# LuckyLYM/Zebra

Measured on AMD Instinct MI355X. Metric: temporal edges/sec embedded (k=20, 2-layer), higher is better.
Workload: dtype f64+f32

## Files before the change

include/zebra_amd.h:

```cpp
#ifndef ZEBRA_AMD_H
#define ZEBRA_AMD_H

#include <stdint.h>

#ifdef __cplusplus
extern "C" {
#endif

#define ZT_OK 0
#define ZT_ERR_ARG (-1)
#define ZT_ERR_RANGE (-2)
#define ZT_ERR_HIP (-3)
#define ZT_ERR_UNSUPPORTED (-4)
#define ZT_ERR_TIMEOUT (-5)

#define ZT_MAX_K 63
#define ZT_MAX_K_WIDE 255

const char *zt_last_error(void);
const char *zt_version(void);

int zt_stream_create_masked(void **stream_out, int32_t cu_lo, int32_t cu_hi);
int zt_stream_destroy(void *stream);

#define ZT_CHOICE_AGGREGATE 0
#define ZT_CHOICE_EMBED_OUT 1
#define ZT_CHOICE_GRU 2
#define ZT_CHOICE_MESSAGES 3
#define ZT_CHOICE_TPPR_CHAIN 4
#define ZT_CHOICE_TPPR_PREPASS 5
#define ZT_CHOICE_GROUP_RELEASE 6
#define ZT_CHOICE_COUNT 7
#define ZT_AGG_GENERIC 1
#define ZT_OUT_TILED 1
#define ZT_OUT_LATENCY 2
#define ZT_OUT_PERSIST 3
#define ZT_GRU_TILE 1
#define ZT_GRU_SPLIT 2
#define ZT_CHAIN_SINGLE 1
#define ZT_CHAIN_PAIRED 2
#define ZT_CHAIN_SPINE 3
#define ZT_CHAIN_DUO 4
#define ZT_PREPASS_LAUNCHES 1
#define ZT_PREPASS_COOP 2
#define ZT_RELEASE_MEMBER 1
#define ZT_RELEASE_LAUNCH 2
#define ZT_RELEASE_LAUNCH_FULL 3
#define ZT_MSG_ONE 1
#define ZT_MSG_TWO 2
int zt_set_kernel_choice(int32_t which, int32_t value);

int zt_profile_enable(int on);
int zt_profile_reset(void);
int zt_profile_read(const char *name, int64_t *count, double *total_ms);


typedef struct zt_tppr zt_tppr;

int zt_tppr_create(zt_tppr **out, int64_t num_nodes, int32_t k, int32_t n_tppr,
                   const double *alpha_host, const double *beta_host);
int zt_tppr_destroy(zt_tppr *h);
int zt_tppr_set_device_share(zt_tppr *h, int32_t n_processes);
int zt_tppr_chain_stats(zt_tppr *h, int64_t *out5, void *stream);

int zt_tppr_reset(zt_tppr *h, void *stream);

int zt_tppr_copy(zt_tppr *dst, const zt_tppr *src, void *stream);

int zt_tppr_stream(zt_tppr *h, const int32_t *nodes_dev, const double *ts_dev,
                   const int64_t *eidx_dev, int64_t B, int32_t n_roles,
                   int32_t emit, int32_t model, int32_t *out_nodes_dev,
                   int32_t *out_eidx_dev, float *out_dt_dev, float *out_w_dev,
                   uint64_t plan_token, void *stream);

int zt_tppr_plan(zt_tppr *h, const int32_t *nodes_dev, const int64_t *eidx_dev,
                 int64_t B, int32_t n_roles, int32_t model, uint64_t *token_out,
                 void *stream);

int zt_tppr_status(zt_tppr *h, void *stream);

int zt_tppr_export(zt_tppr *h, int32_t m, int32_t *len_host, double *norm_host,
                   int64_t *eidx_host, int64_t *node_host, double *ts_host,
                   double *w_host);
int zt_tppr_export_rows(zt_tppr *h, int32_t m, const int64_t *ids_host, int64_t n,
                        int32_t *len_host, double *norm_host, int64_t *eidx_host,
                        int64_t *node_host, double *ts_host, double *w_host);
// ... 266 lines not shown
```

zebra_amd/_capi.py:

```python
import ctypes as C
import os

import torch

_HERE = os.path.dirname(os.path.abspath(__file__))
LIB_PATH = os.path.join(_HERE, "lib", "libzebra_amd.so")

ZT_OK = 0
ZT_ERR_ARG, ZT_ERR_RANGE, ZT_ERR_HIP, ZT_ERR_UNSUPPORTED, ZT_ERR_TIMEOUT = -1, -2, -3, -4, -5

SYMBOLS = [
    "zt_last_error", "zt_version", "zt_set_kernel_choice", "zt_profile_enable", "zt_profile_reset", "zt_profile_read", "zt_stream_create_masked", "zt_stream_destroy",
    "zt_tppr_create", "zt_tppr_destroy", "zt_tppr_set_device_share", "zt_tppr_chain_stats", "zt_tppr_reset", "zt_tppr_copy", "zt_tppr_stream", "zt_tppr_plan", "zt_tppr_status",
    "zt_tppr_export", "zt_tppr_export_rows", "zt_tppr_import", "zt_tppr_import_rows",
    "zt_csr_build", "zt_csr_from_sorted", "zt_csr_size", "zt_csr_export", "zt_csr_destroy", "zt_csr_find_before", "zt_pruned_topk", "zt_pruned_topk_multi",
    "zt_embed_workspace_bytes", "zt_embed", "zt_project_table_bytes", "zt_project_memory", "zt_agg_train_forward", "zt_agg_backward_workspace_bytes", "zt_agg_train_backward", "zt_agg_train_supported", "zt_pipeline_create", "zt_pipeline_destroy", "zt_pipeline_main_stream", "zt_pipeline_update", "zt_pipeline_step", "zt_pipeline_step_ahead", "zt_pipeline_set_group",
    "zt_store_messages", "zt_store_messages_range", "zt_gru_workspace_bytes", "zt_gru_rows_offset", "zt_gru_update", "zt_gemm_f32", "zt_colsum_f32", "zt_overlay_rows", "zt_overlay_rows_backward", "zt_gru_train_workspace_bytes", "zt_gru_train_forward", "zt_gru_train_backward", "zt_pipeline_set_stats", "zt_pipeline_outstanding", "zt_pack_rows", "zt_scatter_rows", "zt_attention_workspace_bytes", "zt_temporal_attention",
    "zt_affinity_workspace_bytes", "zt_affinity", "zt_link_metrics", "zt_pipeline_set_scoring", "zt_pipeline_last_scores", "zt_pipeline_run",
    "zt_exchange_unique_id", "zt_exchange_create", "zt_exchange_set_tables", "zt_exchange_destroy", "zt_pipeline_set_exchange",
    "zt_rnn_update", "zt_rnn_train_forward", "zt_rnn_train_backward", "zt_pipeline_set_cell",
]


CHOICE_AGGREGATE, CHOICE_EMBED_OUT, CHOICE_GRU, CHOICE_MESSAGES, CHOICE_TPPR_CHAIN, CHOICE_TPPR_PREPASS = 0, 1, 2, 3, 4, 5
CHOICE_GROUP_RELEASE = 6
RELEASE_MEMBER, RELEASE_LAUNCH, RELEASE_LAUNCH_FULL = 1, 2, 3
PREPASS_LAUNCHES, PREPASS_COOP = 1, 2
CHAIN_SINGLE, CHAIN_PAIRED, CHAIN_SPINE, CHAIN_DUO = 1, 2, 3, 4
AGG_GENERIC = 1
OUT_TILED, OUT_LATENCY, OUT_PERSIST = 1, 2, 3
GRU_TILE, GRU_SPLIT = 1, 2
CELL_GRU, CELL_RNN = 0, 1
MSG_ONE, MSG_TWO = 1, 2


def set_kernel_choice(which, value):
    check(lib().zt_set_kernel_choice(C.c_int32(which), C.c_int32(value)), "zt_set_kernel_choice")
    _choices[which] = value


_choices = {}


def kernel_choice(which):
    return _choices.get(which, 0)


class RowTables(C.Structure):
    _fields_ = [("ptr", C.c_void_p * 8), ("width", C.c_int32 * 8), ("n", C.c_int32)]


class EmbedWeights(C.Structure):
    _fields_ = [(n, C.c_void_p) for n in ("fc1_w", "fc1_b", "fc2_w", "fc2_b", "fc1s_w", "fc1s_b", "fc2s_w",
                                          "fc2s_b", "time_w")]


class AttnWeights(C.Structure):
    _fields_ = [(n, C.c_void_p) for n in ("q_w", "k_w", "v_w", "in_b", "out_w", "out_b", "m1_w", "m1_b", "m2_w", "m2_b")]


class AffinityWeights(C.Structure):
    _fields_ = [(n, C.c_void_p) for n in ("fc1_w", "fc1_b", "fc2_w", "fc2_b")]


class GruWeights(C.Structure):
    _fields_ = [(n, C.c_void_p) for n in ("w_ih", "w_hh", "b_ih", "b_hh")]


class PipelineDesc(C.Structure):
    _fields_ = [("tppr", C.c_void_p), ("csr", C.c_void_p), ("width", C.c_int32), ("depth", C.c_int32),
                ("alpha", C.c_double * 16), ("beta", C.c_double * 16),
                ("memory", C.c_void_p), ("last_update", C.c_void_p), ("messages", C.c_void_p), ("msg_ts", C.c_void_p),
                ("flags", C.c_void_p), ("scratch", C.c_void_p), ("efeat", C.c_void_p),
                ("num_nodes", C.c_int64), ("num_edges", C.c_int64),
                ("D", C.c_int32), ("F", C.c_int32), ("T", C.c_int32), ("M", C.c_int32), ("k", C.c_int32),
                ("ew", EmbedWeights), ("gw", GruWeights),
                ("embed_ws", C.c_void_p), ("gru_ws", C.c_void_p), ("proj_table", C.c_void_p), ("status", C.c_void_p),
                ("max_B", C.c_int64)]


XCHG_RCCL, XCHG_SHM = 1, 2

# ... 96 lines not shown
```

zebra_amd/csrc/aggregate.hip:

```cpp
#include "common.hpp"
#include "embed_out_body.hpp"

using namespace zt;

namespace {

constexpr int MAX_MT = 5;
constexpr int MAX_MT_BIG = 16;
constexpr int MAX_MT_BIG_WIDE = 8;
constexpr int LDS_BUDGET = 150 * 1024;

__host__ __device__ inline int round_up(int x, int m) { return (x + m - 1) / m * m; }

#ifdef ZT_AGG_STAMP
__device__ unsigned long long g_agg[8];
#define AGG_STAMP(i) do { if (threadIdx.x == 0) { const long long t__ = clock64(); atomicAdd(&g_agg[i], (unsigned long long)(t__ - t_prev__)); t_prev__ = t__; } } while (0)
#else
#define AGG_STAMP(i) do { } while (0)
#endif

__global__ void k_pad_matrix(const float *__restrict__ W, int ld, int c0, int rows, int cols, float *__restrict__ Wp,
                             int rows_p, int cols_p)
{
    const int i = blockIdx.x * blockDim.x + threadIdx.x;
// ... 766 lines not shown
                            acc[b] = __builtin_amdgcn_mfma_f32_16x16x4f32(A_cur[u], Breg[b][st0 + u], acc[b], 0, 0, 0);
                }
#pragma unroll
                for (int u = 0; u < 2; ++u) {
                    const int st = st0 + u;
                    if (!(a > 0 && st < REG_NB)) continue;
                    const int b = st;
                    float part = 0.f;
#pragma unroll
                    for (int j = 0; j < 4; ++j) {
                        float v = accv[b][j] + ((DBG & 2) ? 0.f : Pv[ap & 1][b][j]);
                        v = v > 0.f ? v : 0.f;
                        part += (DBG & 2) ? v : v * wn_prv[j];
                    }
                    if (DBG & 2) {
                        Hloc[q_lo][b] += part;
                    } else {
                        const int pi = __float_as_int(part);
                        const auto h = __builtin_amdgcn_permlane32_swap(pi, pi, false, false);
                        const auto lo = __builtin_amdgcn_permlane16_swap(h[0], h[0], false, false);
                        const auto hi = __builtin_amdgcn_permlane16_swap(h[1], h[1], false, false);
                        const float pg[4] = {__int_as_float(lo[0]), __int_as_float(lo[1]), __int_as_float(hi[0]), __int_as_float(hi[1])};
#pragma unroll
                        for (int g = 0; g < 4; ++g) {
                            const int q = (16 * ap + 4 * g) / KK;
                            if (q < RQ) Hloc[q][b] += pg[g];
                        }
                    }
                    asm volatile("" : "+v"(Hloc[q_lo][b]));
                    if (q_hi != q_lo && q_hi < RQ) asm volatile("" : "+v"(Hloc[q_hi][b]));
                }
                if (a >= 1 && a <= 3 && st0 == REG_NB + 1 && !(DBG & 4)) load_P(a + 1);
                __builtin_amdgcn_sched_barrier(0);
            }
        }
#pragma unroll
        for (int q = 0; q < RQ; ++q) {
            if (g4 == (q & 3) && q < nq) {
                float *hrow = H + ((size_t)m * N + q0 + q) * D;
#pragma unroll
                for (int b = 0; b < REG_NB; ++b)
                    if (16 * b + r16 < D) hrow[16 * b + r16] = Hloc[q][b];
            }
        }
        wave_sync();
    }
#ifdef ZT_DIAG
    if (DBG && lane == 0 && blockIdx.x * AGG_WAVES + wave < 1024) {
        unsigned long long *o = g_regclk + 4 * (blockIdx.x * AGG_WAVES + wave);
        o[0] = __builtin_amdgcn_s_memtime() - clk0; o[1] = wall0; o[2] = __builtin_amdgcn_s_memrealtime();
        o[3] = wall_in;
    }
#endif
}


constexpr int EO3_NT = 7, EO3_KC = 7, EO3_DP = 112, EO3_LDY = 116;
constexpr int EO3_FRAG = EO3_NT * EO3_KC * 256;

__device__ __forceinline__ void eo3_fill(float *Wl, const float *__restrict__ Wp, int tid)
{
    constexpr int PER = (EO3_NT * EO3_KC * 64 + 255) / 256;
    f32x4 v[PER];
#pragma unroll
    for (int q = 0; q < PER; ++q) {
        const int idx = tid + q * 256, frag = idx >> 6, ln = idx & 63;
        const int b = frag / EO3_KC, c = frag - b * EO3_KC;
        v[q] = idx < EO3_NT * EO3_KC * 64
                   ? *reinterpret_cast<const f32x4 *>(Wp + (size_t)(16 * b + (ln & 15)) * EO3_DP + 16 * c + 4 * (ln >> 4))
                   : f32x4{0.f, 0.f, 0.f, 0.f};
    }
#pragma unroll
    for (int q = 0; q < PER; ++q) {
        const int idx = tid + q * 256;
        if (idx < EO3_NT * EO3_KC * 64) reinterpret_cast<f32x4 *>(Wl)[idx] = v[q];
    }
}

template <int HG>
__global__ __launch_bounds__(AGG_THREADS, 1) void k_embed_out3(
    const float *__restrict__ memory, long long num_nodes, const int *__restrict__ nodes, long long N, int D, int M,
    const float *__restrict__ H, const float *__restrict__ S, const float *__restrict__ fc2_p,
    const float *__restrict__ fc2_b, const float *__restrict__ fc1s_p, const float *__restrict__ fc1s_b,
    const float *__restrict__ fc2s_p, const float *__restrict__ fc2s_b, float *__restrict__ out, int *status, int n_src)
{
    extern __shared__ __attribute__((aligned(16))) char smem[];
    float *W0 = reinterpret_cast<float *>(smem);
    const int tid = threadIdx.x, lane = tid & 63, wave = tid >> 6, r16 = lane & 15, g4 = lane >> 4;
    const int OW = D * (M + 1);
    const long long tiles = (N + 15) / 16;
    const f32x4 zero4 = {0.f, 0.f, 0.f, 0.f};
    bool cin[EO3_KC];
#pragma unroll
    for (int c = 0; c < EO3_KC; ++c) cin[c] = 16 * c + 4 * g4 < D;
    const f32x4 *Wf0 = reinterpret_cast<const f32x4 *>(W0) + lane;

    if ((int)blockIdx.x < n_src) {
        float *W1 = W0 + EO3_FRAG;
        float *Y = W1 + EO3_FRAG + wave * 16 * EO3_LDY;
        eo3_fill(W0, fc1s_p, tid);
        eo3_fill(W1, fc2s_p, tid);
        float b1v[EO3_NT], b2v[EO3_NT];
#pragma unroll
        for (int b = 0; b < EO3_NT; ++b) {
            b1v[b] = 16 * b + r16 < D ? fc1s_b[16 * b + r16] : 0.f;
            b2v[b] = 16 * b + r16 < D ? fc2s_b[16 * b + r16] : 0.f;
// ... 192 lines not shown
{
    const int lda = Kp + 4;
    int mt = max_mt;
    while (mt > 1 && ((size_t)mt * 16 * lda * 4 + (size_t)mt * 16 * 16) > (size_t)LDS_BUDGET) --mt;
    int rq = (mt * 16) / k;
    if (rq < 1) {
        mt = (k + 15) / 16;
        rq = 1;
        if (mt > max_mt || ((size_t)mt * 16 * lda * 4 + (size_t)mt * 16 * 16) > (size_t)LDS_BUDGET) return false;
    }
    mt = (rq * k + 15) / 16;
    if ((size_t)mt * 16 * (Dp + 1) * 4 > (size_t)mt * 16 * lda * 4) return false;
    *lda_out = lda; *mt_out = mt; *rq_out = rq;
    *lds_out = (size_t)mt * 16 * lda * 4 + (size_t)mt * 16 * 16 + (size_t)T * 4;
    return true;
}

bool split_fits(int D, int F, int T, int k) { return k <= ZT_MAX_K_WIDE && fc1_agg_split_rows(D, F, T) > 0; }

bool make_plan(int64_t N, int D, int F, int T, int M, int k, EmbedPlan &p)
{
    if (!width_supported(D)) return false;
    const int K1 = D + F + T;
    p.Dp = round_up(D, 16);
    p.K1p = round_up(K1, 16);
    const bool big = k > MAX_MT * 16;
    const int max_mt = big ? (p.Dp > 16 * NTW * AGG_WAVES ? MAX_MT_BIG_WIDE : MAX_MT_BIG) : MAX_MT;
    const bool full_ok = tile_shape(p.K1p, p.Dp, k, T, &p.lda, &p.mt, &p.rq, &p.lds, max_mt);
    if (!full_ok) { p.mt = 0; p.rq = 1; p.lda = p.K1p + 4; p.lds = 0; }
    p.K2p = round_up(F + T, 16);
    p.mt2 = 0;
    if (!(full_ok || big) || !tile_shape(p.K2p, p.Dp, k, T, &p.lda2, &p.mt2, &p.rq2, &p.lds2, max_mt)) p.mt2 = 0;
    if (p.mt == 0 && p.mt2 == 0 && !split_fits(D, F, T, k)) return false;
    size_t o = 0;
    auto take = [&](size_t bytes) { size_t r = o; o += (bytes + 255) & ~(size_t)255; return r; };
    p.off_w1p = take((size_t)p.Dp * p.K1p * 4);
    p.off_fc2t = take((size_t)p.Dp * p.Dp * 4);
    p.off_fc1st = take((size_t)p.Dp * p.Dp * 4);
    p.off_fc2st = take((size_t)p.Dp * p.Dp * 4);
    p.off_w1t = take((size_t)p.Dp * p.K2p * 4);
    p.off_wm = take((size_t)p.Dp * p.Dp * 4);
    p.hg = fc1_agg_wide_supported(D, F, T, k) ? k / 4 : 1;
    p.off_wl = take(p.hg > 1 ? fc1_agg_wide_weight_bytes() : 0);
    p.off_wfrag = take((size_t)REG_FRAG_GROUPS * 64 * 4 * 4);
    p.off_H = take((size_t)M * N * D * 4 * p.hg);
    p.off_S = take((size_t)M * N * 4);
    p.total = o;
    return true;
}

KernelPlan plan_kernels(int64_t N, int D, int F, int T, int M, int k, bool have_table, bool training, int agg_choice,
                        int out_choice, EmbedPlan &p)
{
    KernelPlan kp{AggKernel::unsupported, OutForm::tiled, Refusal::shape, 0, 0, 0, 0, 1};
    static_assert(16 * NTW * AGG_WAVES == 128 && 16 * NTW_WIDE * AGG_WAVES == MAX_D, "the N-tiles cover D <= 128 / D <= 256");
    if (!make_plan(N, D, F, T, M, k, p)) return kp;
    const bool big = k > MAX_MT * 16;
    const bool tab = have_table && !training && p.mt2 > 0;
    const bool special = tab && agg_choice != ZT_AGG_GENERIC;
    if (training ? (big || p.mt == 0) : (!tab && p.mt == 0)) {
        if (!split_fits(D, F, T, k)) { kp.refusal = Refusal::no_split; return kp; }
        kp.agg = AggKernel::split;
    } else if (special && p.hg > 1) {
        kp.agg = AggKernel::wide;
    } else if (special && D == 100 && T == 100 && F <= 4 && (k == 20 || k == 40) && p.K2p == 112) {
        kp.agg = AggKernel::reg;
    } else if (special && D == 100 && T == 100 && p.mt2 == 5 && (k == 10 || k == 20 || k == 40)) {
        kp.agg = AggKernel::d100;
    } else if (tab) {
        kp.agg = big ? AggKernel::tiled_table_big : AggKernel::tiled_table;
    } else {
        kp.agg = big ? AggKernel::tiled_full_big : AggKernel::tiled_full;
    }
    if (kp.agg == AggKernel::d100 || kp.agg == AggKernel::tiled_table || kp.agg == AggKernel::tiled_table_big) {
        kp.lds = p.lds2; kp.rq = p.rq2; kp.mt = p.mt2; kp.lda = p.lda2;
    } else if (kp.agg == AggKernel::tiled_full || kp.agg == AggKernel::tiled_full_big) {
        kp.lds = p.lds; kp.rq = p.rq; kp.mt = p.mt; kp.lda = p.lda;
    }
    kp.hg = kp.agg == AggKernel::wide ? p.hg : 1;
    if (kp.hg != 1 && kp.hg != 5 && kp.hg != 10) { kp.agg = AggKernel::unsupported; kp.refusal = Refusal::groups; return kp; }
    kp.refusal = Refusal::none;
    if (D % 4 == 0 && (p.Dp == 112 || p.Dp == 128) && (out_choice == ZT_OUT_LATENCY || (out_choice == 0 && N <= 1024)))
        kp.out = OutForm::latency;
    else if (D % 4 == 0 && p.Dp == EO3_DP && (out_choice == ZT_OUT_PERSIST || (out_choice == 0 && N >= 8192)))
        kp.out = OutForm::persist;
    return kp;
}

}

KernelPlan zt::embed_kernel_plan(int64_t N, int D, int F, int T, int M, int k, bool have_table, bool training, int agg_choice,
                                 int out_choice)
{
    EmbedPlan p;
    return plan_kernels(N, D, F, T, M, k, have_table, training, agg_choice, out_choice, p);
}

#ifdef ZT_AGG_STAMP
extern "C" int zt_debug_agg(unsigned long long *host, int reset)
{
    ZT_HIP(hipDeviceSynchronize());
    ZT_HIP(hipMemcpyFromSymbol(host, HIP_SYMBOL(g_agg), sizeof(unsigned long long) * 8));
    if (reset) { unsigned long long z[8] = {0}; ZT_HIP(hipMemcpyToSymbol(HIP_SYMBOL(g_agg), z, sizeof(z))); }
    return ZT_OK;
}
#endif

#ifdef ZT_DIAG
extern "C" int zt_debug_regclk(unsigned long long *host)
{
    ZT_HIP(hipDeviceSynchronize());
    ZT_HIP(hipMemcpyFromSymbol(host, HIP_SYMBOL(g_regclk), sizeof(unsigned long long) * 4 * 1024));
    return ZT_OK;
}
#endif

extern "C" int64_t zt_embed_workspace_bytes(int64_t N, int32_t D, int32_t F, int32_t T, int32_t M, int32_t k)
{
    EmbedPlan p;
// ... 83 lines not shown
    if (N == 0) return ZT_OK;
    if (!nodes_dev || !nbr_dev || !eix_dev || !dt_dev || !w_dev || !out_dev || !workspace_dev) {
        set_error("zt_embed: NULL buffer");
        return ZT_ERR_ARG;
    }
    EmbedPlan p;
    const KernelPlan kp = plan_kernels(N, D, F, T, M, k, proj_table_dev != nullptr, false, kernel_choice(ZT_CHOICE_AGGREGATE),
                                       kernel_choice(ZT_CHOICE_EMBED_OUT), p);
    if (kp.refusal == Refusal::shape) {
        set_error("zt_embed: D=%d F=%d T=%d k=%d outside the supported shapes (D <= 128, or a multiple of 4 up to %d; one query "
                  "row of k neighbours must fit the %d KB LDS tile)", D, F, T, k, MAX_D, LDS_BUDGET / 1024);
        return ZT_ERR_UNSUPPORTED;
    }
    hipStream_t s = (hipStream_t)stream;
    char *ws = reinterpret_cast<char *>(workspace_dev);
    float *H = reinterpret_cast<float *>(ws + p.off_H);
    float *S = reinterpret_cast<float *>(ws + p.off_S);
    if (!weights_ready) {
        ZT_PROF_BEGIN(s, P_EMBED_PREP);
        embed_prepare(wt, D, F, T, p, ws, s);
        ZT_PROF_END(s, P_EMBED_PREP);
    }
    if (kp.refusal == Refusal::no_split) {
        set_error("zt_embed: k=%d needs the projected table (a query row's [memory | ef | time] tile does not fit %d KB of LDS, "
                  "nor does a chunk of it)", k, LDS_BUDGET / 1024);
        return ZT_ERR_UNSUPPORTED;
    }
    if (kp.refusal == Refusal::groups) { set_error("zt_embed: %d partial-sum groups per row", kp.hg); return ZT_ERR_UNSUPPORTED; }
    const bool waits_inside = kp.agg == AggKernel::wide || kp.agg == AggKernel::reg;
    if (gate != nullptr && gate->word != nullptr && !waits_inside) {
        const int rc = zt::member_gate_launch(*gate, status_dev, s);
        if (rc != ZT_OK) return rc;
    }
    const dim3 tile_grid((unsigned)(kp.rq > 0 ? (N + kp.rq - 1) / kp.rq : 0), (unsigned)M);
    const bool wide = p.Dp > 16 * NTW * AGG_WAVES;
    auto tiled = [&](decltype(&k_fc1_agg<false>) fn, const float *rows, int ld, size_t w_off, int Kp) {
        ZT_HIP(set_dynamic_lds(reinterpret_cast<const void *>(fn), kp.lds));
        fn<<<tile_grid, AGG_THREADS, kp.lds, s>>>(rows, efeat_dev, wt->time_w, num_nodes, num_edges, ld, F, T, N, k, kp.rq, kp.mt,
                                                  kp.lda, nbr_dev, eix_dev, dt_dev, w_dev, reinterpret_cast<const float *>(ws + w_off),
                                                  Kp, wt->fc1_b, H, S, status_dev, D, nullptr, nullptr, 0u, 0u, 0u, 1.f);
        return ZT_OK;
    };
    auto reg = [&](decltype(&k_fc1_agg_reg<20>) fn) {
        const long long rq = 80 / k, tiles = ((N + rq - 1) / rq) * M;
        long long wgs = (tiles + AGG_WAVES - 1) / AGG_WAVES;
        const int cus = stream_cu_count(s);
        if (wgs > cus) wgs = cus;
        fn<<<(unsigned)wgs, AGG_THREADS, 0, s>>>(proj_table_dev, efeat_dev, wt->time_w, num_nodes, num_edges, F, N, M, nbr_dev, eix_dev,
                                                 dt_dev, w_dev, reinterpret_cast<const float *>(ws + p.off_wfrag), wt->fc1_b, H, S,
                                                 status_dev, gate ? gate->word : nullptr, gate ? gate->target : 0,
                                                 gate ? gate->latch : nullptr);
        return ZT_OK;
    };
    ZT_PROF_BEGIN(s, P_FC1_AGG);
    int rc = ZT_OK;
    switch (kp.agg) {
    case AggKernel::wide:
        rc = fc1_agg_wide_launch(proj_table_dev, efeat_dev, wt->time_w, num_nodes, num_edges, N, M, k, nbr_dev, eix_dev, dt_dev,
                                 w_dev, reinterpret_cast<const float *>(ws + p.off_wl), wt->fc1_b, H, S, status_dev,
                                 stream_cu_count(s), s, gate);
        break;
    case AggKernel::reg:
#ifdef ZT_DIAG
        {
            static const int dbg = getenv("ZT_AGG_DBG") ? atoi(getenv("ZT_AGG_DBG")) : 0;
            if (k == 20 && dispatch<1, 2, 6, 7, 8>(dbg, [&](auto DB) { return reg(k_fc1_agg_reg<20, DB>); }) == ZT_OK) break;
        }
#endif
        rc = dispatch<20, 40>(k, [&](auto KK) { return reg(k_fc1_agg_reg<KK>); });
        break;
    case AggKernel::d100:
        rc = dispatch<10, 20, 40>(k, [&](auto KK) {
            ZT_HIP(set_dynamic_lds(reinterpret_cast<const void *>(k_fc1_agg_d100<KK>), kp.lds));
            k_fc1_agg_d100<KK><<<tile_grid, AGG_THREADS, kp.lds, s>>>(proj_table_dev, efeat_dev, wt->time_w, num_nodes, num_edges, F, N,
                                                                     kp.lda, nbr_dev, eix_dev, dt_dev, w_dev,
                                                                     reinterpret_cast<const float *>(ws + p.off_w1t), p.K2p, wt->fc1_b,
                                                                     H, S, status_dev);
            return ZT_OK;
        });
        break;
    case AggKernel::tiled_table:
        rc = tiled(wide ? k_fc1_agg<true, MAX_MT, NTW_WIDE> : k_fc1_agg<true>, proj_table_dev, p.Dp, p.off_w1t, p.K2p);
        break;
    case AggKernel::tiled_table_big:
        rc = tiled(wide ? k_fc1_agg<true, MAX_MT_BIG_WIDE, NTW_WIDE> : k_fc1_agg<true, MAX_MT_BIG>, proj_table_dev, p.Dp, p.off_w1t,
                   p.K2p);
        break;
    case AggKernel::tiled_full: rc = tiled(wide ? k_fc1_agg<false, MAX_MT, NTW_WIDE> : k_fc1_agg<false>, memory_dev, D, p.off_w1p, p.K1p); break;
    case AggKernel::tiled_full_big:
        rc = tiled(wide ? k_fc1_agg<false, MAX_MT_BIG_WIDE, NTW_WIDE> : k_fc1_agg<false, MAX_MT_BIG>, memory_dev, D, p.off_w1p, p.K1p);
        break;
    case AggKernel::split:
        rc = fc1_agg_split_launch(memory_dev, nullptr, nullptr, efeat_dev, wt->time_w, num_nodes, num_edges, D, F, T, N, M, k,
                                  nbr_dev, eix_dev, dt_dev, w_dev, reinterpret_cast<const float *>(ws + p.off_w1p), p.K1p,
                                  wt->fc1_b, H, S, status_dev, 0.f, 0ull, s);
        break;
    case AggKernel::unsupported: break;
    }
    if (rc != ZT_OK) return rc;
    ZT_PROF_END(s, P_FC1_AGG);
    if (mid_wait != nullptr) ZT_HIP(hipStreamWaitEvent(s, mid_wait, 0));
    const EmbedOutArgs E{memory_dev, num_nodes, nodes_dev, N, D, M, H, S,
                         reinterpret_cast<const float *>(ws + p.off_fc2t), wt->fc2_b,
                         reinterpret_cast<const float *>(ws + p.off_fc1st), wt->fc1s_b,
                         reinterpret_cast<const float *>(ws + p.off_fc2st), wt->fc2s_b, out_dev, status_dev};
    const long long tiles = (N + 15) / 16;
    const zt::embed_out_deferred od{true, E, kp.hg, kp.out, kp.out == OutForm::latency ? (int)(tiles < 256 ? tiles : 256) : 0, nullptr};
    if (defer != nullptr && kp.out != OutForm::persist) {
        int *latch = defer->latch;
        *defer = od;
        defer->latch = latch;
        ZT_LAUNCH_CHECK();
        return ZT_OK;
    }
    ZT_PROF_BEGIN(s, P_EMBED_OUT);
    rc = zt::embed_out_launch(od, s);
    if (rc != ZT_OK) return rc;
    ZT_PROF_END(s, P_EMBED_OUT);
    ZT_LAUNCH_CHECK();
    return ZT_OK;
}

// ... 125 lines not shown
```

zebra_amd/csrc/common.hpp:

```cpp
#pragma once

#include <hip/hip_runtime.h>

#include <cstdint>
#include <cstdio>
#include <cstdlib>
#include <type_traits>

#include "../../include/zebra_amd.h"

namespace zt {

void set_error(const char *fmt, ...);

enum ProfId { P_PREPASS = 0, P_STREAM, P_CLEANUP, P_PRUNE, P_EMBED_PREP, P_FC1_AGG, P_EMBED_OUT, P_STORE_MSG, P_GRU,
              P_SCORE, P_EXCHANGE, P_COUNT };
extern bool g_prof_on;
void prof_begin(hipStream_t s, int id);
void prof_end(hipStream_t s, int id);
int tppr_stream_ex(zt_tppr *h, const int32_t *nodes_dev, const double *ts_dev, const int64_t *eidx_dev, int64_t B,
                   int32_t n_roles, int32_t emit, int32_t model, int32_t *out_nodes_dev, int32_t *out_eidx_dev,
                   float *out_dt_dev, float *out_w_dev, uint64_t plan_token, void *stream, bool plan_ordered,
                   hipEvent_t *done_out, int32_t sub_B, int32_t *member_done_dev = nullptr);
constexpr int TPPR_MAX_MEMBERS = 8;
constexpr int TPPR_MEMBER_WORDS = TPPR_MAX_MEMBERS + 1;
struct EmbedOutArgs {
    const float *memory;
    long long num_nodes;
    const int *nodes;
    long long N;
    int D, M;
    const float *H, *S, *fc2_p, *fc2_b, *fc1s_p, *fc1s_b, *fc2s_p, *fc2s_b;
    float *out;
    int *status;
};
enum class AggKernel { unsupported, reg, wide, d100, tiled_table, tiled_full, tiled_table_big, tiled_full_big, split };
enum class OutForm { tiled, latency, persist };
enum class Refusal { none, shape, no_split, groups };
struct KernelPlan {
    AggKernel agg;
    OutForm out;
    Refusal refusal;
    size_t lds;
    int rq, mt, lda;
    int hg;
};
KernelPlan embed_kernel_plan(int64_t N, int D, int F, int T, int M, int k, bool have_table, bool training, int agg_choice,
                             int out_choice);
enum class MsgKernel { one, two };
enum class GruForm { none, tile, split };
enum class OutLaunch { none, front, fused_tile, fused_split };
enum class MemRefusal { none, arg, d_large, msg_wide };
struct HeldOut {
    bool present;
    OutForm form;
    int hg, D, M, gx;
    long long N;
    bool same_memory;
};
struct MemoryPlan {
    MsgKernel msg;
    GruForm gru;
    OutLaunch out;
    MemRefusal refusal;
    size_t lds, lds2, lds_f;
    int gru_tiles, NTg;
    int n_src_wgs, n_nb_wgs, out_tiles;
    unsigned grid;
    unsigned target, participants;
};
MemoryPlan memory_kernel_plan(int64_t max_rows, int D, int msg_dim, int F, int T, int gru_choice, int msg_choice,
                              const HeldOut &held);
struct embed_out_deferred {
    bool valid;
    EmbedOutArgs args;
    int hg;
    OutForm form;
    int gx;
    int *latch;
};
int embed_out_launch(const embed_out_deferred &d, void *stream);
int gru_update_ex(float *memory_dev, float *last_update_dev, const float *messages_dev, const float *msg_ts_dev,
                  uint8_t *flags_dev, int64_t num_nodes, int32_t D, int32_t msg_dim, const int32_t *ids_dev, int64_t n_ids,
                  const int32_t *n_ids_dev, const zt_gru_weights *wt, void *workspace_dev, int32_t weights_ready,
                  const float *wm_p, float *proj_table, void *stream, bool counter_zeroed = false, bool select_done = false,
                  embed_out_deferred *fuse = nullptr, int cell = ZT_CELL_GRU);
int store_messages_ex(const float *memory_dev, const float *last_update_dev, const float *efeat_dev, const float *time_w_dev,
                      int64_t num_nodes, int64_t num_edges, int32_t D, int32_t F, int32_t T, const int32_t *src_dev,
                      const int32_t *dst_dev, const double *ts_dev, const int64_t *eidx_dev, int64_t B, int64_t pos_lo,
                      int64_t pos_hi, float *messages_dev, float *msg_ts_dev, uint8_t *flags_dev, int32_t *scratch_dev,
                      int32_t *uniq_ids_dev, int32_t *n_uniq_dev, int32_t *status_dev, int32_t *zero_word_dev, void *stream,
                      bool *zeroed_out = nullptr, bool set_flags = true);
struct member_gate {
    const int32_t *word;
    int32_t target;
    int *latch;
};
int member_gate_launch(const member_gate &g, int32_t *status_dev, void *stream);
// ... 256 lines not shown
```

Before: 13.39 million.

## Add shared-entry register aggregation kernel that dedups repeated neighbor slots across roles

Adds a new fc1 aggregate kernel for D=100, T=100, k=20/40 that groups two query roles per wave-unit, detects neighbor slots in the second role identical to live slots in the first, and computes the fc1 MFMA only for unique live entries, compacted via ballot. Results are staged in LDS and reused in the weighted sum, with prefetching of the next unit's indices and edge features overlapping compute. It becomes the default when M<=2, with a new choice value to fall back to the plain register kernel. The added LDS staging, ballot compaction and a persistent grid capped at the CU count add overhead that pays off only when many entries are zero-weight or duplicated.

```diff
diff --git a/include/zebra_amd.h b/include/zebra_amd.h
--- a/include/zebra_amd.h
+++ b/include/zebra_amd.h
@@ -32,6 +32,7 @@
 #define ZT_CHOICE_GROUP_RELEASE 6
 #define ZT_CHOICE_COUNT 7
 #define ZT_AGG_GENERIC 1
+#define ZT_AGG_REG_PLAIN 2
 #define ZT_OUT_TILED 1
 #define ZT_OUT_LATENCY 2
 #define ZT_OUT_PERSIST 3
diff --git a/zebra_amd/_capi.py b/zebra_amd/_capi.py
--- a/zebra_amd/_capi.py
+++ b/zebra_amd/_capi.py
@@ -28,6 +28,7 @@
 PREPASS_LAUNCHES, PREPASS_COOP = 1, 2
 CHAIN_SINGLE, CHAIN_PAIRED, CHAIN_SPINE, CHAIN_DUO = 1, 2, 3, 4
 AGG_GENERIC = 1
+AGG_REG_PLAIN = 2
 OUT_TILED, OUT_LATENCY, OUT_PERSIST = 1, 2, 3
 GRU_TILE, GRU_SPLIT = 1, 2
 CELL_GRU, CELL_RNN = 0, 1
diff --git a/zebra_amd/csrc/aggregate.hip b/zebra_amd/csrc/aggregate.hip
--- a/zebra_amd/csrc/aggregate.hip
+++ b/zebra_amd/csrc/aggregate.hip
@@ -842,6 +842,305 @@
         o[3] = wall_in;
     }
 #endif
+}
+
+constexpr int REGS_PITCH = 100;
+constexpr int REGS_MAX_M = 2;
+struct __attribute__((aligned(16))) RegsLds {
+    int nb[80], ei[80];
+    float dt[80], w[80], ef[80 * 4];
+    int e_nb[80];
+    float e_dt[80], e_ef[80 * 4];
+    int ent[80];
+    float sum[4];
+    float stage[80 * REGS_PITCH];
+};
+static_assert(sizeof(RegsLds) % 16 == 0 && AGG_WAVES * sizeof(RegsLds) <= 160 * 1024, "four waves' buffers in one CU's LDS");
+
+template <int KK>
+__global__ __launch_bounds__(AGG_THREADS, 1) void k_fc1_agg_regs(
+    const float *__restrict__ P, const float *__restrict__ efeat, const float *__restrict__ time_w, long long num_nodes,
+    long long num_edges, int F, long long N, int M, const int *__restrict__ nbr, const int *__restrict__ eix,
+    const float *__restrict__ dt, const float *__restrict__ w, const float *__restrict__ Wfrag,
+    const float *__restrict__ b1, float *__restrict__ H, float *__restrict__ S, int *status,
+    const int *gate_word, int gate_target, int *gate_latch)
+{
+    constexpr int D = 100, T = 100, DP = 112, ROWS = 80, RQ = ROWS / KK, PITCH = REGS_PITCH;
+    static_assert(KK % 4 == 0 && ROWS % KK == 0 && RQ % REGS_MAX_M == 0, "groups of 4 slots must not straddle query rows");
+    extern __shared__ __attribute__((aligned(16))) char smem[];
+    const int lane = threadIdx.x & 63, wave = threadIdx.x >> 6;
+    const int r16 = lane & 15, g4 = lane >> 4;
+    RegsLds &L = reinterpret_cast<RegsLds *>(smem)[wave];
+
+    float Breg[REG_NB][REG_NS];
+    {
+        const f32x4 *Wf = reinterpret_cast<const f32x4 *>(Wfrag) + lane;
+        constexpr int HB = REG_FRAG_GROUPS / 2;
+#pragma unroll
+        for (int half = 0; half < 2; ++half) {
+            f32x4 v[HB];
+#pragma unroll
+            for (int i = 0; i < HB; ++i) v[i] = Wf[(half * HB + i) * 64];
+            __builtin_amdgcn_sched_barrier(0);
+#pragma unroll
+            for (int i = 0; i < HB; ++i)
+#pragma unroll
+                for (int e = 0; e < 4; ++e) {
+                    const int q = 4 * (half * HB + i) + e;
+                    if (q < REG_NB * REG_NS) asm volatile("v_accvgpr_write_b32 %0, %1" : "=a"(Breg[q / REG_NS][q % REG_NS]) : "v"(v[i][e]));
+                }
+            __builtin_amdgcn_sched_barrier(0);
+        }
+    }
+    float freq[REG_NS];
+#pragma unroll
+    for (int st = 0; st < REG_NS; ++st) {
+        const int kc = 4 * st + g4 - F;
+        freq[st] = (kc >= 0 && kc < T) ? time_w[kc] : 0.f;
+    }
+    float bias[REG_NB];
+#pragma unroll
+    for (int b = 0; b < REG_NB; ++b) bias[b] = (16 * b + r16) < D ? b1[16 * b + r16] : 0.f;
+
+    const bool two = M == 2;
+    const int UQ = two ? RQ / 2 : RQ;
+    const long long n_units = (N + UQ - 1) / UQ;
+    const long long stride = (long long)gridDim.x * AGG_WAVES;
+    long long unit = (long long)blockIdx.x * AGG_WAVES + wave;
+
+    int pf_nb[2] = {0, 0}, pf_ei[2] = {0, 0};
+    float pf_dt[2] = {0.f, 0.f}, pf_w[2] = {0.f, 0.f};
+    auto fetch = [&](long long u) {
+        const long long q0 = u * UQ;
+        int ln = lane;
+        asm volatile("" : "+v"(ln));
+#pragma unroll
+        for (int h = 0; h < 2; ++h) {
+            const int row = h * 64 + ln;
+            const int r = row / KK, j = row - r * KK;
+            const int m = (two && r >= RQ / 2) ? 1 : 0, q = r - m * UQ;
+            const bool in = (h == 0 || lane < ROWS - 64) && q0 + q < N;
+            const size_t ix = in ? (((size_t)m * N + q0 + q) * KK + j) : 0;
+            pf_nb[h] = in ? nbr[ix] : 0;
+            pf_ei[h] = in ? eix[ix] : 0;
+            pf_dt[h] = in ? dt[ix] : 0.f;
+            pf_w[h] = in ? w[ix] : 0.f;
+        }
+    };
+    float pf_ef[2][4] = {{0.f, 0.f, 0.f, 0.f}, {0.f, 0.f, 0.f, 0.f}};
+    auto fetch_ef = [&]() {
+#pragma unroll
+        for (int h = 0; h < 2; ++h) {
+            const int ei = pf_ei[h];
+            const bool ok = ei >= 0 && ei < num_edges && (h == 0 || lane < ROWS - 64);
+#pragma unroll
+            for (int c = 0; c < 4; ++c) pf_ef[h][c] = (ok && c < F) ? efeat[(size_t)ei * F + c] : 0.f;
+        }
+    };
+    member_gate_enter(gate_word, gate_target, status, gate_latch);
+    if (unit < n_units) { fetch(unit); fetch_ef(); }
+
+#pragma nounroll
+    for (; unit < n_units; unit += stride) {
+        const long long q0 = unit * UQ;
+        int nbv[2], eiv[2];
+#pragma unroll
+        for (int h = 0; h < 2; ++h) {
+            const int row = h * 64 + lane;
+            nbv[h] = pf_nb[h]; eiv[h] = pf_ei[h];
+            if (h == 0 || lane < ROWS - 64) {
+                if (nbv[h] < 0 || nbv[h] >= num_nodes || eiv[h] < 0 || eiv[h] >= num_edges) { atomicExch(status, ZT_ERR_RANGE); nbv[h] = 0; eiv[h] = 0; }
+                L.nb[row] = nbv[h]; L.ei[row] = eiv[h]; L.dt[row] = pf_dt[h]; L.w[row] = pf_w[h];
+                *reinterpret_cast<f32x4 *>(L.ef + 4 * row) = f32x4{pf_ef[h][0], pf_ef[h][1], pf_ef[h][2], pf_ef[h][3]};
+            }
+        }
+        wave_sync();
+        if (lane < RQ) {
+            f32x4 wv[KK / 4];
+#pragma unroll
+            for (int j = 0; j < KK / 4; ++j) wv[j] = *reinterpret_cast<const f32x4 *>(L.w + lane * KK + 4 * j);
+            float sm = 0.f;
+#pragma unroll
+            for (int j = 0; j < KK; ++j) sm += wv[j / 4][j % 4];
+            L.sum[lane] = sm;
+            const int m = (two && lane >= RQ / 2) ? 1 : 0, q = lane - m * UQ;
+            if (q0 + q < N) S[(size_t)m * N + q0 + q] = (sm == 0.f) ? 0.f : 1.f;
+        }
+        wave_sync();
+        float wn[2] = {0.f, 0.f};
+#pragma unroll
+        for (int h = 0; h < 2; ++h) {
+            const int row = h * 64 + lane;
+            if (h == 0 || lane < ROWS - 64) {
+                const float qs = L.sum[row / KK];
+                wn[h] = (qs == 0.f) ? 0.f : pf_w[h] / qs;
+                L.w[row] = wn[h];
+            }
+        }
+        wave_sync();
+        if (two && lane < ROWS / 2) {
+            const int slot = ROWS / 2 + lane, base = (lane / KK) * KK;
+            const int mn = L.nb[slot], me = L.ei[slot], md = __float_as_int(L.dt[slot]);
+            int mt = -1;
+#pragma unroll
+            for (int jj = KK / 4 - 1; jj >= 0; --jj) {
+                const int4 n4 = *reinterpret_cast<const int4 *>(L.nb + base + 4 * jj);
+                const int4 e4 = *reinterpret_cast<const int4 *>(L.ei + base + 4 * jj);
+                const int4 d4 = *reinterpret_cast<const int4 *>(L.dt + base + 4 * jj);
+                const f32x4 w4 = *reinterpret_cast<const f32x4 *>(L.w + base + 4 * jj);
+                if (n4.w == mn && e4.w == me && d4.w == md && w4[3] != 0.f) mt = base + 4 * jj + 3;
+                if (n4.z == mn && e4.z == me && d4.z == md && w4[2] != 0.f) mt = base + 4 * jj + 2;
+                if (n4.y == mn && e4.y == me && d4.y == md && w4[1] != 0.f) mt = base + 4 * jj + 1;
+                if (n4.x == mn && e4.x == me && d4.x == md && w4[0] != 0.f) mt = base + 4 * jj;
+            }
+            L.ent[slot] = mt;
+        }
+        wave_sync();
+        bool live[2], isE[2];
+        int match[2], ent[2];
+#pragma unroll
+        for (int h = 0; h < 2; ++h) {
+            const int slot = h * 64 + lane;
+            const bool valid = h == 0 || lane < ROWS - 64;
+            live[h] = valid && wn[h] != 0.f;
+            match[h] = (two && valid && slot >= ROWS / 2 && live[h]) ? L.ent[slot] : -1;
+            isE[h] = live[h] && match[h] < 0;
+        }
+        const unsigned long long mask0 = __ballot(isE[0]), mask1 = __ballot(isE[1]);
+        const int n0 = __popcll(mask0), n_ent = n0 + __popcll(mask1);
+        const int n_mt = n_ent > 16 ? (n_ent + 15) >> 4 : 1;
+        ent[0] = (int)__builtin_amdgcn_mbcnt_hi((unsigned)(mask0 >> 32), __builtin_amdgcn_mbcnt_lo((unsigned)mask0, 0u));
+        ent[1] = n0 + (int)__builtin_amdgcn_mbcnt_hi((unsigned)(mask1 >> 32), __builtin_amdgcn_mbcnt_lo((unsigned)mask1, 0u));
+        wave_sync();
+#pragma unroll
+        for (int h = 0; h < 2; ++h) {
+            if (isE[h]) {
+                const int e = ent[h];
+                L.ent[h * 64 + lane] = e;
+                L.e_nb[e] = nbv[h]; L.e_dt[e] = pf_dt[h];
+                *reinterpret_cast<f32x4 *>(L.e_ef + 4 * e) = f32x4{pf_ef[h][0], pf_ef[h][1], pf_ef[h][2], pf_ef[h][3]};
+            }
+        }
+        if (n_ent + lane < 16 * n_mt) {
+            const int e = n_ent + lane;
+            L.e_nb[e] = 0; L.e_dt[e] = 0.f;
+            *reinterpret_cast<f32x4 *>(L.e_ef + 4 * e) = f32x4{0.f, 0.f, 0.f, 0.f};
+        }
+        wave_sync();
+#pragma unroll
+        for (int h = 0; h < 2; ++h)
+            if (!isE[h]) ent[h] = match[h] >= 0 ? L.ent[match[h]] : -1;
+        const bool has_next = unit + stride < n_units;
+        if (has_next) fetch(unit + stride);
+
+        f32x4 acc[REG_NB];
+        float accv[REG_NB][4], Pv[2][REG_NB][4];
+        auto load_P = [&](int x, auto SETC) {
+            constexpr int SET = decltype(SETC)::value;
+            const int4 nb4 = *reinterpret_cast<const int4 *>(L.e_nb + x * 16 + 4 * g4);
+            const float *p0 = P + (size_t)nb4.x * DP + r16, *p1 = P + (size_t)nb4.y * DP + r16,
+                        *p2 = P + (size_t)nb4.z * DP + r16, *p3 = P + (size_t)nb4.w * DP + r16;
+#pragma unroll
+            for (int b = 0; b < REG_NB; ++b) {
+                Pv[SET][b][0] = p0[16 * b]; Pv[SET][b][1] = p1[16 * b]; Pv[SET][b][2] = p2[16 * b]; Pv[SET][b][3] = p3[16 * b];
+            }
+        };
+        using set0 = std::integral_constant<int, 0>;
+        using set1 = std::integral_constant<int, 1>;
+        load_P(0, set0{});
+        if (n_mt > 1) load_P(1, set1{});
+        auto round = [&](int a, auto SETC, auto MFC, auto EPC) {
+            constexpr int SET = decltype(SETC)::value;
+            constexpr bool MF = decltype(MFC)::value, EP = decltype(EPC)::value;
+            float dta = 0.f, A_next[2] = {0.f, 0.f};
+            if (EP) {
+#pragma unroll
+                for (int b = 0; b < REG_NB; ++b)
+#pragma unroll
+                    for (int j = 0; j < 4; ++j) accv[b][j] = acc[b][j];
+            }
+            if (MF) {
+                dta = L.e_dt[a * 16 + r16];
+                const float ef = L.e_ef[4 * (a * 16 + r16) + (g4 & 3)];
+#pragma unroll
+                for (int b = 0; b < REG_NB; ++b) acc[b] = f32x4{bias[b], bias[b], bias[b], bias[b]};
+                A_next[0] = time_cosf_rev(dta * freq[0]);
+                A_next[1] = time_cosf_rev(dta * freq[1]);
+                if (g4 < F) A_next[0] = ef;
+            }
+            __builtin_amdgcn_sched_barrier(0);
+#pragma unroll
+            for (int st0 = 0; st0 < REG_NS; st0 += 2) {
+                if (!MF && st0 >= REG_NB) break;
+                const float A_cur[2] = {A_next[0], A_next[1]};
+                if (MF) {
+#pragma unroll
+                    for (int u = 0; u < 2; ++u)
+                        if (st0 + 2 + u < REG_NS) A_next[u] = time_cosf_rev(dta * freq[st0 + 2 + u]);
+#pragma unroll
+                    for (int u = 0; u < 2; ++u)
+#pragma unroll
+                        for (int b = 0; b < REG_NB; ++b)
+                            acc[b] = __builtin_amdgcn_mfma_f32_16x16x4f32(A_cur[u], Breg[b][st0 + u], acc[b], 0, 0, 0);
+                }
+#pragma unroll
+                for (int u = 0; u < 2; ++u) {
+                    const int b = st0 + u;
+                    if (!(EP && b < REG_NB)) continue;
+                    if (16 * b + r16 < D) {
+                        float *sp = L.stage + (16 * (a - 1) + 4 * g4) * PITCH + 16 * b + r16;
+#pragma unroll
+                        for (int j = 0; j < 4; ++j) {
+                            const float v = accv[b][j] + Pv[SET ^ 1][b][j];
+                            sp[j * PITCH] = v > 0.f ? v : 0.f;
+                        }
+                    }
+                }
+                if (MF && EP && st0 == REG_NB + 1 && a + 1 < n_mt) load_P(a + 1, std::integral_constant<int, (SET ^ 1)>{});
+                __builtin_amdgcn_sched_barrier(0);
+            }
+        };
+        round(0, set0{}, std::true_type{}, std::false_type{});
+        if (has_next) fetch_ef();
+        for (int a = 1;; a += 2) {
+            if (a < n_mt) round(a, set1{}, std::true_type{}, std::true_type{});
+            else { round(a, set1{}, std::false_type{}, std::true_type{}); break; }
+            if (a + 1 < n_mt) round(a + 1, set0{}, std::true_type{}, std::true_type{});
+            else { round(a + 1, set0{}, std::false_type{}, std::true_type{}); break; }
+        }
+        wave_sync();
+
+        int lr = lane;
+        asm volatile("" : "+v"(lr));
+        const int c1 = 64 + (lr < D - 64 ? lr : D - 65);
+#pragma unroll
+        for (int r = 0; r < RQ; ++r) {
+            float h0 = 0.f, h1 = 0.f;
+#pragma unroll
+            for (int g = 0; g < KK / 4; ++g) {
+                float part0 = 0.f, part1 = 0.f;
+#pragma unroll
+                for (int j = 0; j < 4; ++j) {
+                    const int s = r * KK + 4 * g + j;
+                    const int e = __builtin_amdgcn_readlane(ent[s >> 6], s & 63);
+                    const float wv = __int_as_float(__builtin_amdgcn_readlane(__float_as_int(wn[s >> 6]), s & 63));
+                    const float *row = L.stage + (e > 0 ? e : 0) * PITCH;
+                    const float v0 = row[lr], v1 = row[c1];
+                    part0 = e >= 0 ? part0 + v0 * wv : part0;
+                    part1 = e >= 0 ? part1 + v1 * wv : part1;
+                }
+                h0 += part0; h1 += part1;
+            }
+            const int m = (two && r >= RQ / 2) ? 1 : 0, q = r - m * UQ;
+            if (q0 + q < N) {
+                float *hrow = H + ((size_t)m * N + q0 + q) * D;
+                hrow[lr] = h0;
+                if (lr < D - 64) hrow[64 + lr] = h1;
+            }
+            __builtin_amdgcn_sched_barrier(0);
+        }
+        wave_sync();
+    }
 }
 
 
@@ -1140,7 +1439,7 @@
 KernelPlan plan_kernels(int64_t N, int D, int F, int T, int M, int k, bool have_table, bool training, int agg_choice,
                         int out_choice, EmbedPlan &p)
 {
-    KernelPlan kp{AggKernel::unsupported, OutForm::tiled, Refusal::shape, 0, 0, 0, 0, 1};
+    KernelPlan kp{AggKernel::unsupported, OutForm::tiled, Refusal::shape, 0, 0, 0, 0, 1, false};
     static_assert(16 * NTW * AGG_WAVES == 128 && 16 * NTW_WIDE * AGG_WAVES == MAX_D, "the N-tiles cover D <= 128 / D <= 256");
     if (!make_plan(N, D, F, T, M, k, p)) return kp;
     const bool big = k > MAX_MT * 16;
@@ -1153,6 +1452,7 @@
         kp.agg = AggKernel::wide;
     } else if (special && D == 100 && T == 100 && F <= 4 && (k == 20 || k == 40) && p.K2p == 112) {
         kp.agg = AggKernel::reg;
+        kp.reg_shared = agg_choice != ZT_AGG_REG_PLAIN && M <= REGS_MAX_M;
     } else if (special && D == 100 && T == 100 && p.mt2 == 5 && (k == 10 || k == 20 || k == 40)) {
         kp.agg = AggKernel::d100;
     } else if (tab) {
@@ -1342,6 +1642,19 @@
                                                  gate ? gate->latch : nullptr);
         return ZT_OK;
     };
+    auto regs = [&](decltype(&k_fc1_agg_regs<20>) fn) {
+        const long long uq = 80 / (k * M), units = (N + uq - 1) / uq;
+        long long wgs = (units + AGG_WAVES - 1) / AGG_WAVES;
+        const int cus = stream_cu_count(s);
+        if (wgs > cus) wgs = cus;
+        const size_t lds = AGG_WAVES * sizeof(RegsLds);
+        ZT_HIP(set_dynamic_lds(reinterpret_cast<const void *>(fn), lds));
+        fn<<<(unsigned)wgs, AGG_THREADS, lds, s>>>(proj_table_dev, efeat_dev, wt->time_w, num_nodes, num_edges, F, N, M, nbr_dev, eix_dev,
+                                                   dt_dev, w_dev, reinterpret_cast<const float *>(ws + p.off_wfrag), wt->fc1_b, H, S,
+                                                   status_dev, gate ? gate->word : nullptr, gate ? gate->target : 0,
+                                                   gate ? gate->latch : nullptr);
+        return ZT_OK;
+    };
     ZT_PROF_BEGIN(s, P_FC1_AGG);
     int rc = ZT_OK;
     switch (kp.agg) {
@@ -1357,7 +1670,8 @@
             if (k == 20 && dispatch<1, 2, 6, 7, 8>(dbg, [&](auto DB) { return reg(k_fc1_agg_reg<20, DB>); }) == ZT_OK) break;
         }
 #endif
-        rc = dispatch<20, 40>(k, [&](auto KK) { return reg(k_fc1_agg_reg<KK>); });
+        if (kp.reg_shared) rc = dispatch<20, 40>(k, [&](auto KK) { return regs(k_fc1_agg_regs<KK>); });
+        else rc = dispatch<20, 40>(k, [&](auto KK) { return reg(k_fc1_agg_reg<KK>); });
         break;
     case AggKernel::d100:
         rc = dispatch<10, 20, 40>(k, [&](auto KK) {
diff --git a/zebra_amd/csrc/common.hpp b/zebra_amd/csrc/common.hpp
--- a/zebra_amd/csrc/common.hpp
+++ b/zebra_amd/csrc/common.hpp
@@ -44,6 +44,7 @@
     size_t lds;
     int rq, mt, lda;
     int hg;
+    bool reg_shared;
 };
 KernelPlan embed_kernel_plan(int64_t N, int D, int F, int T, int M, int k, bool have_table, bool training, int agg_choice,
                              int out_choice);
```

New measurement: 11.98 million. 0.895x the previous value.
